# 30hours/blah2

Measured on AMD Instinct MI355X. Metric: CPIs/s, higher is better.
Workload: dtype f32; 1 GPU; BASELINE configs[1]: 2 MS/s, 1 s CPI, +-256 Hz -> 513 Doppler x 411 delay bins, synthetic c32 IQ resident in HBM; chain=amb, fmt=c32, n_samples=2000000, fs=2000000, n_doppler_bins=513, n_delay_bins=411, n_corr=3898, fft_len=1024, n_seg=7, seg_len=576, doppler_kernel=tile16, prewarm_steps=252, range_kernel=wave1k, ring_batches=2, streams_per_gpu=1

## Files before the change

blah2_amd/csrc/capi.hip:

```cpp
#include "kernels.hpp"
#include "cfar_kernels.hpp"
#include "timing.hpp"

#include <algorithm>
#include <cmath>
#include <complex>
#include <cstdio>
#include <cstdlib>
#include <cstring>
#include <deque>
#include <map>
#include <mutex>
#include <set>
#include <string>
#include <vector>

using namespace blah2;

namespace {

thread_local std::string g_err;

int fail(int code, const std::string &msg)
{
// ... 33 lines not shown
  int32_t delayMin = 0, delayMax = 0, dopplerMin = 0, dopplerMax = 0;
  uint32_t fs = 0;
  int r3 = 8;
  RangePlan plan{};
  struct LagChunk { int32_t lag0, count, col0; };
  std::vector<LagChunk> chunks;
  int32_t maxChunk = 0;
  std::vector<int32_t> delayAxis;
  std::vector<double> dopplerAxis;
  hipStream_t stream = nullptr;
  int numCU = 256;
  int rangeGridForce = 0;
  int rangeGridLast = 0;
  void *h_pin = nullptr;
  size_t h_pin_bytes = 0;

  cf *d_tw = nullptr;
  cf *d_dopW = nullptr;
  double2 *d_dopW64 = nullptr;
  uint32_t *d_hotCount = nullptr;
  cf *d_R = nullptr;
  cf *d_map = nullptr;
  double *d_partSum = nullptr;
  uint32_t *d_tickets = nullptr;
  float *d_partMax = nullptr;
  double *d_metrics = nullptr;
  double *d_doppler = nullptr;
  void *d_in = nullptr;
  size_t d_in_bytes = 0;
  cf *d_rot = nullptr;
  blah2hip_hit_t *d_hits = nullptr;
  uint32_t *d_count = nullptr;
  uint32_t hitCap = 0;
  int dopTilesX = 0, dopTilesY = 0;
  int dopR3 = 0;
  int dopGridX = 0;
  int nParts = 0;
  int nTiles = 0;
  int dopForce = BLAH2HIP_DOP_AUTO;
  int lastDoppler = 0;
  int lastRange = 0;
  int rangeKernel = 0;
  int fftLenForce = 0;
  int cfar2dForce = 0;
  int dopGridForce = 0;
  int dopGridLast = 0, dopTilesLast = 0;
// ... 303 lines not shown
  const bool out7 = a.plan.nDelay <= 7 * 64;
  auto kern = shortx ? (out7 ? rangeps_kernel<In, true, true> : rangeps_kernel<In, true, false>)
                     : (out7 ? rangeps_kernel<In, false, true> : rangeps_kernel<In, false, false>);
  LDSCFG(kern, lds);
  const int grid = std::min<int>(a.nPulses, range_grid_cap(h, lds, RANGEPS_WAVES, 12));
  hipLaunchKernelGGL(kern, dim3(grid), dim3(64 * RANGEPS_WAVES), lds, st, a, in);
  HIPCHK(hipGetLastError());
  h->lastRange = BLAH2HIP_RANGE_PS;
  return BLAH2HIP_OK;
}

template <class In> int launch_range(blah2hip_amb_s *h, const RangeArgs &a, In in, hipStream_t st)
{
  if (use_wave_range(h, a.nPulses)) return launch_rangew_t(h, a, in, st);
  if (use_wave1k_range(h, a.nPulses)) return launch_rangew1k_t(h, a, in, st);
  if (use_ps_range(h, a.nPulses)) return launch_rangeps_t(h, a, in, st);
  switch (h->r3) {
  case 4: return launch_range8_t<2>(h, a, in, st);
  case 8: return launch_range_t<8>(h, a, in, st);
  default: return launch_range_t<16>(h, a, in, st);
  }
}

int upload_range_table(blah2hip_amb_s *h)
{
  const int F = (int)h->dims.fft_len;
  std::vector<cf> tw(F);
  for (int k = 0; k < F; k++) tw[k] = root_of_unity(k, F);
  if (h->d_tw) HIPCHK(hipFree(h->d_tw));
  h->d_tw = nullptr;
  HIPCHK(hipMalloc(&h->d_tw, F * sizeof(cf)));
  HIPCHK(hipMemcpy(h->d_tw, tw.data(), F * sizeof(cf), hipMemcpyHostToDevice));
  return BLAH2HIP_OK;
}

int tic(blah2hip_amb_s *h, int k, hipStream_t st)
{
  HIPCHK(h->timer.tic(k, st));
  return BLAH2HIP_OK;
}

int toc(blah2hip_amb_s *h, int k, hipStream_t st)
{
  HIPCHK(h->timer.toc(k, st));
  return BLAH2HIP_OK;
}
// ... 604 lines not shown
    HIPCHK(hipMemcpy(h->d_chirp, chirp.data(), chirp.size() * sizeof(cf), hipMemcpyHostToDevice));
    HIPCHK(hipMemcpy(h->d_bf, bf.data(), bf.size() * sizeof(cf), hipMemcpyHostToDevice));
  }
  return BLAH2HIP_OK;
  };
  const int rc = build();
  if (rc != BLAH2HIP_OK) {
    blah2hip_amb_destroy(h);
    return rc;
  }
  *out = h;
  return BLAH2HIP_OK;
}

int blah2hip_amb_destroy(blah2hip_amb_t h)
{
  if (!h) return BLAH2HIP_OK;
  (void)hipSetDevice(h->device);
  if (h->stream) (void)hipStreamSynchronize(h->stream);
  for (void *p : {(void *)h->d_tw, (void *)h->d_dopW, (void *)h->d_R, (void *)h->d_map,
                  (void *)h->d_partSum, (void *)h->d_partMax, (void *)h->d_tickets, (void *)h->d_metrics,
                  (void *)h->d_doppler, h->d_in, (void *)h->d_rot,
                  (void *)h->d_hits, (void *)h->d_count, (void *)h->d_sat, (void *)h->d_dtw, (void *)h->d_chirp,
                  (void *)h->d_bf, (void *)h->d_bfn, (void *)h->d_H, (void *)h->d_dopW64, (void *)h->d_hotCount, (void *)h->d_firK0})
    if (p) (void)hipFree(p);
  for (auto &t : h->alphaTables)
    if (t.d) (void)hipFree(t.d);
  if (h->h_pin) (void)hipHostFree(h->h_pin);
  leak_clear(h);
  h->timer.destroy();
  if (h->stream) (void)hipStreamDestroy(h->stream);
  delete h;
  return BLAH2HIP_OK;
}

int blah2hip_amb_get_dims(blah2hip_amb_t h, blah2hip_amb_dims_t *dims)
{
  if (!h || !dims) return fail(BLAH2HIP_ERR_INVALID, "NULL argument");
  *dims = h->dims;
  return BLAH2HIP_OK;
}

int blah2hip_amb_get_axes(blah2hip_amb_t h, int32_t *delay, double *doppler)
{
  if (!h) return fail(BLAH2HIP_ERR_INVALID, "NULL handle");
  if (delay) std::memcpy(delay, h->delayAxis.data(), h->delayAxis.size() * sizeof(int32_t));
  if (doppler) std::memcpy(doppler, h->dopplerAxis.data(), h->dopplerAxis.size() * sizeof(double));
// ... 89 lines not shown
int blah2hip_amb_get_info(blah2hip_amb_t h, int key, int64_t *value)
{
  if (!h || !value) return fail(BLAH2HIP_ERR_INVALID, "NULL argument");
  switch (key) {
  case BLAH2HIP_INFO_LAST_DOPPLER_KERNEL: *value = h->lastDoppler; return BLAH2HIP_OK;
  case BLAH2HIP_INFO_LAST_RANGE_KERNEL: *value = h->lastRange; return BLAH2HIP_OK;
  case BLAH2HIP_INFO_DOPPLER_FFT_LEN: *value = 256 * h->dopR3; return BLAH2HIP_OK;
  case BLAH2HIP_INFO_RANGE_GRID: *value = h->rangeGridLast; return BLAH2HIP_OK;
  case BLAH2HIP_INFO_NUM_CU: *value = h->numCU; return BLAH2HIP_OK;
  case BLAH2HIP_INFO_DOPPLER_GRID: *value = h->dopGridLast; return BLAH2HIP_OK;
  case BLAH2HIP_INFO_DOPPLER_TILES: *value = h->dopTilesLast; return BLAH2HIP_OK;
  case BLAH2HIP_INFO_LEAK_LAGS: *value = h->lastLeakLags; return BLAH2HIP_OK;
  case BLAH2HIP_INFO_LEAK_MAX_E12: *value = (int64_t)std::llround(h->lastLeakMax * 1e12); return BLAH2HIP_OK;
  case BLAH2HIP_INFO_HOT_COLUMNS: {
    *value = 0;
    if (!h->lastHot) return BLAH2HIP_OK;
    uint32_t n = 0;
    HIPCHK(hipSetDevice(h->device));
    HIPCHK(hipMemcpyAsync(&n, h->d_hotCount, sizeof(n), hipMemcpyDeviceToHost, h->lastHotStream));
    HIPCHK(hipStreamSynchronize(h->lastHotStream));
    *value = n;
    return BLAH2HIP_OK;
  }
  case BLAH2HIP_INFO_HOT_COLUMNS_MISSED: {
    *value = 0;
    if (!h->lastHot) return BLAH2HIP_OK;
    std::vector<uint32_t> n(h->lastHotCpis);
    HIPCHK(hipSetDevice(h->device));
    HIPCHK(hipMemcpyAsync(n.data(), h->d_hotCount + h->dims.max_batch, n.size() * sizeof(uint32_t), hipMemcpyDeviceToHost,
                          h->lastHotStream));
    HIPCHK(hipStreamSynchronize(h->lastHotStream));
    for (uint32_t v : n) *value = std::max<int64_t>(*value, v);
    return BLAH2HIP_OK;
  }
  default: return fail(BLAH2HIP_ERR_INVALID, "unknown info key");
  }
}

int blah2hip_amb_process_dev(blah2hip_amb_t h, int fmt, const void *d_x, const void *d_y,
                             uint32_t n_cpi, uint64_t cpi_stride, void *d_map, double *d_metrics,
                             void *stream)
{
  if (!h) return fail(BLAH2HIP_ERR_INVALID, "NULL handle");
  if (n_cpi == 0 || n_cpi > h->dims.max_batch) return fail(BLAH2HIP_ERR_INVALID, "n_cpi outside [1, max_batch]");
  if (fmt != BLAH2HIP_FMT_C32 && fmt != BLAH2HIP_FMT_I16 && fmt != BLAH2HIP_FMT_F16 && fmt != BLAH2HIP_FMT_I16X_C32Y)
    return fail(BLAH2HIP_ERR_INVALID, "unknown sample format");
// ... 19 lines not shown
  if (h->leakMode != 0 && !h->inLeakCal && !fused) {
    const int rid = predict_range(h, (int)(n_cpi * nD)), did = pick_doppler(h, n_cpi);
    auto it = h->leak.find(rid * 64 + did);
    if (it == h->leak.end()) {
      blah2hip_amb_s::LeakCal cal;
      const int rcc = leak_calibrate(h, rid, did, st, &cal);
      if (rcc) return rcc;
      it = h->leak.emplace(rid * 64 + did, cal).first;
    }
    h->lastLeakMax = it->second.maxAbs;
    if (it->second.nLags > 0 && (it->second.active || h->leakMode == 2)) leak = &it->second;
  }
  if (!h->inLeakCal) h->lastLeakLags = leak ? leak->nLags : 0;

  RangeArgs ra;
  ra.plan = h->plan;
  ra.tw = h->d_tw;
  ra.out = h->d_R;
  ra.cpiStride = (int64_t)cpi_stride;
  ra.nPulses = (int32_t)(n_cpi * nD);

  const int32_t m2 = h->dopplerMin + h->dopplerMax;
  int rc;
  if (m2 != 0) {
    const size_t plane = (size_t)h->dims.n_samples;
    if (!h->d_rot) HIPCHK(hipMalloc(&h->d_rot, 2 * plane * h->dims.max_batch * sizeof(cf)));
    cf *xo = h->d_rot, *yo = h->d_rot + plane * h->dims.max_batch;
    const uint32_t nrot = h->dims.n_used;
    dim3 grid(std::min<uint32_t>((nrot + 255) / 256, 2048), n_cpi);
    if ((rc = tic(h, BLAH2HIP_K_ROTATE, st))) return rc;
    if (fmt == BLAH2HIP_FMT_C32) {
      InC32 in{(const cf *)d_x, (const cf *)d_y};
      hipLaunchKernelGGL(rotate_kernel<InC32>, grid, dim3(256), 0, st, in, xo, yo,
                         (int64_t)cpi_stride, (int64_t)plane, nrot, m2, h->fs);
    } else if (fmt == BLAH2HIP_FMT_F16) {
      InF16 in{(const _Float16 *)d_x, (const _Float16 *)d_y};
      hipLaunchKernelGGL(rotate_kernel<InF16>, grid, dim3(256), 0, st, in, xo, yo,
                         (int64_t)cpi_stride, (int64_t)plane, nrot, m2, h->fs);
    } else if (fmt == BLAH2HIP_FMT_I16X_C32Y) {
      InI16C32 in{(const int16_t *)d_x, (const cf *)d_y};
      hipLaunchKernelGGL(rotate_kernel<InI16C32>, grid, dim3(256), 0, st, in, xo, yo,
                         (int64_t)cpi_stride, (int64_t)plane, nrot, m2, h->fs);
    } else {
      InI16 in{(const int16_t *)d_x};
      hipLaunchKernelGGL(rotate_kernel<InI16>, grid, dim3(256), 0, st, in, xo, yo,
                         (int64_t)cpi_stride, (int64_t)plane, nrot, m2, h->fs);
// ... 13 lines not shown
    using W = WgFft<16>;
    const size_t lds = (size_t)(W::A_ELEMS + W::B_ELEMS) * sizeof(cf);
    LDSCFG(taps_spectrum_kernel, lds);
    hipLaunchKernelGGL(taps_spectrum_kernel, dim3(n_cpi), dim3(256), lds, st, h->firW, h->firBins, h->d_tw, h->d_H, h->d_firK0);
    RangeFirArgs fa;
    fa.plan = h->plan;
    fa.plan.delayMin = h->chunks[0].lag0; fa.plan.nDelay = h->chunks[0].count; fa.plan.colOff = h->chunks[0].col0;
    fa.tw = h->d_tw; fa.out = h->d_R; fa.cpiStride = (int64_t)cpi_stride; fa.nPulses = (int32_t)(n_cpi * nD);
    fa.H = h->d_H; fa.N = h->dims.n_samples; fa.w = h->firW; fa.nBins = h->firBins; fa.k0 = h->d_firK0;
    const size_t ldsf = lds + 240 * sizeof(cf);
    const int grid = std::min<int>(fa.nPulses, range_grid_cap(h, ldsf, 4, 8));
    if (fmt == BLAH2HIP_FMT_C32) {
      InC32 in{(const cf *)d_x, (const cf *)d_y};
      LDSCFG(range_fir_kernel<InC32>, ldsf);
      hipLaunchKernelGGL(range_fir_kernel<InC32>, dim3(grid), dim3(256), ldsf, st, fa, in);
    } else {
      InI16 in{(const int16_t *)d_x};
      LDSCFG(range_fir_kernel<InI16>, ldsf);
      hipLaunchKernelGGL(range_fir_kernel<InI16>, dim3(grid), dim3(256), ldsf, st, fa, in);
    }
    HIPCHK(hipGetLastError());
    h->lastRange = BLAH2HIP_RANGE_FIR;
    if ((rc = toc(h, BLAH2HIP_K_RANGE, st))) return rc;
  } else {
    if ((rc = tic(h, BLAH2HIP_K_RANGE, st))) return rc;
    for (const auto &ck : h->chunks) {
      ra.plan.delayMin = ck.lag0; ra.plan.nDelay = ck.count; ra.plan.colOff = ck.col0;
      if (fmt == BLAH2HIP_FMT_C32) {
        InC32 in{(const cf *)d_x, (const cf *)d_y};
        rc = launch_range(h, ra, in, st);
      } else if (fmt == BLAH2HIP_FMT_F16) {
        InF16 in{(const _Float16 *)d_x, (const _Float16 *)d_y};
        rc = launch_range(h, ra, in, st);
      } else if (fmt == BLAH2HIP_FMT_I16X_C32Y) {
        InI16C32 in{(const int16_t *)d_x, (const cf *)d_y};
        rc = launch_range(h, ra, in, st);
      } else {
        InI16 in{(const int16_t *)d_x};
        rc = launch_range(h, ra, in, st);
      }
      if (rc) return rc;
    }
    if ((rc = toc(h, BLAH2HIP_K_RANGE, st))) return rc;
  }

  DopplerArgs da;
  da.R = h->d_R;
  da.map = map;
  da.W = h->d_dopW;
  da.tw = h->d_dtw;
  da.chirp = h->d_chirp;
  da.bf = h->d_bf;
  da.bfn = h->d_bfn;
  da.partSum = h->d_partSum;
  da.partMax = h->d_partMax;
  da.nD = (int32_t)nD;
  da.nDelay = (int32_t)nDelay;
  da.nTiles = h->nTiles;
  int nPartsUsed = 0, dopGrid = 0, dopTiles = 0;
  if ((rc = tic(h, BLAH2HIP_K_DOPPLER, st))) return rc;
  const int which = pick_doppler(h, n_cpi);
  switch (which) {
  case BLAH2HIP_DOP_TILE8:
  case BLAH2HIP_DOP_TILE8K:
  case BLAH2HIP_DOP_TILE16WG:
  case BLAH2HIP_DOP_TILE16: {
    const int ncol = (which == BLAH2HIP_DOP_TILE8 || which == BLAH2HIP_DOP_TILE8K) ? 8 : 16;
    const int grid = (int)((nDelay + ncol - 1) / ncol);
    if (which == BLAH2HIP_DOP_TILE16) {
      const size_t lds = (size_t)DOPT1K_LDS_ELEMS * sizeof(cf);
      const int wgs = (int)std::min<int64_t>((int64_t)grid * n_cpi, h->dopGridForce ? h->dopGridForce : h->numCU);
      dopGrid = wgs; dopTiles = grid * (int)n_cpi;
      LDSCFG(doppler_tile1k_kernel<16>, lds);
      hipLaunchKernelGGL(doppler_tile1k_kernel<16>, dim3(wgs), dim3(1024), lds, st, da, (int)n_cpi);
    } else if (which == BLAH2HIP_DOP_TILE8K) {
      const size_t lds = (size_t)dopt1k_lds_elems<8>() * sizeof(cf);
      const int wgs = (int)std::min<int64_t>((int64_t)grid * n_cpi, h->dopGridForce ? h->dopGridForce : 2 * h->numCU);
      dopGrid = wgs; dopTiles = grid * (int)n_cpi;
      LDSCFG(doppler_tile1k_kernel<8>, lds);
      hipLaunchKernelGGL(doppler_tile1k_kernel<8>, dim3(wgs), dim3(512), lds, st, da, (int)n_cpi);
    } else if (ncol == 16) {
      const size_t lds = (size_t)dopt_lds_elems<16>() * sizeof(cf);
      const int wgs = (int)std::min<int64_t>((int64_t)grid * n_cpi, h->dopGridForce ? h->dopGridForce : h->numCU);
      dopGrid = wgs; dopTiles = grid * (int)n_cpi;
      LDSCFG(doppler_tile_kernel<16>, lds);
// ... 753 lines not shown
```

blah2_amd/csrc/kernels.hpp:

```cpp
#pragma once

#include <hip/hip_runtime.h>

#include "blah2hip.h"
#include "range_core.hpp"
#include "fft_wg8.hpp"
#include "fft_wave.hpp"
#include "fft_wave2.hpp"
#include "fft_wave1k.hpp"
#include "bufload.hpp"
#include "trace.hpp"

namespace blah2 {

#ifndef RANGE8_WAVES_PER_SIMD
#define RANGE8_WAVES_PER_SIMD 3
#endif
struct RangeArgs {
  RangePlan plan;
  const cf *tw;
  cf *out;
  int64_t cpiStride;
  int32_t nPulses;
};
// ... 410 lines not shown
  const int cnt = min(p.segLen, p.nCorr - s0);
  const b2_v4i xd = make_rsrc(B::xp(in, pulseBase + s0), cnt * CX::STRIDE);
  const b2_v4i yd = make_rsrc(B::yp(in, pulseBase), p.nCorr * CY::STRIDE);
  int vx[1] = {t * CX::STRIDE};
  int vy[NV];
#pragma unroll
  for (int j = 0; j < NV; j++) vy[j] = (s0 + p.delayMin + t) * CY::STRIDE + j * 4096;
  typename CX::raw xr[NX];
  typename CY::raw yr[NY];
  bufload_chan<CX, STEPX, NX, true>(xr, xd, vx);
  bufload_chan<CY, STEPY, NY, false>(yr, yd, vy);
  bufwait<NY + NX - 16, 16>(xr);
  if constexpr (NX == 32) bufwait<NY, 16>(xr + 16);
  else bufwait<NY, 8>(xr + 16);
#pragma unroll
  for (int k = 0; k < NX; k++) v[k] = CX::cvt(xr[k]);
  bufwait<NY - 16, 16>(yr);
  if constexpr (NY == 32) bufwait<0, 16>(yr + 16);
  else { bufwait<4, 8>(yr + 16); bufwait<0, 4>(yr + 24); }
#pragma unroll
  for (int k = 0; k < NY; k++) yv[k] = CY::cvt(yr[k]);
}

template <int NC>
__device__ __forceinline__ void store_lags_w(cf *out, const RangePlan &p, int cpi, int pulse, int t, const cf *v)
{
  const int jt = t + (p.colOff & 15);
  cf *o = out + (((int64_t)cpi * p.nTilesOut + (p.colOff >> 4) + (jt >> 4)) * p.nDoppler + pulse) * 16 + (jt & 15);
  const int64_t step = (int64_t)p.nDoppler * 64;
  int rem = p.nDelay - t;
  int nd = p.nDelay;
  asm volatile("" : "+v"(rem), "+s"(nd));
#pragma unroll
  for (int c = 0; c < NC; c++) {
    if (64 * c >= nd) break;
#if defined(RW_NO_STORE)
    if (64 * c < rem && p.scale == 12345.f) *o = cmake(v[c].x * p.scale, v[c].y * p.scale);
#else
    if (64 * c < rem) *o = cmake(v[c].x * p.scale, v[c].y * p.scale);
#endif
    o += step;
  }
}

#ifdef RANGEW_TRACE
#define RW_T(k) { const uint64_t now_ = __builtin_amdgcn_s_memtime(); tr[k] += now_ - t0_; t0_ = now_; }
#else
#define RW_T(k)
#endif

#ifndef RANGEW_WAVES
#define RANGEW_WAVES 8
#endif
template <class In, bool SHORTW, bool OUT7 = SHORTW>
__global__ __launch_bounds__(64 * RANGEW_WAVES, RANGEW_WAVES_PER_SIMD) void rangew_kernel(RangeArgs a, In in)
{
  using W = WaveFft;
  extern __shared__ __attribute__((aligned(16))) char smem[];
  cf *table = reinterpret_cast<cf *>(smem);
  const int t = threadIdx.x & 63;
  const int wave = __builtin_amdgcn_readfirstlane(threadIdx.x >> 6);
  cf *X = table + W::TW_ELEMS + wave * W::X_ELEMS;
// ... 71 lines not shown
  const int s0 = s * p.segLen;
  const int cnt = live ? min(p.segLen, p.nCorr - s0) : 0;
  const __amdgpu_buffer_rsrc_t d = make_rsrc_b(BufLoad<In>::xp(in, pulseBase + s0), cnt * CX::STRIDE);
#pragma unroll
  for (int k = 0; k < NX; k++) rx[k] = RawBuiltin<CX>::ld(d, t * CX::STRIDE, k * 64 * CX::STRIDE);
}
template <class In, int K0 = 0>
__device__ __forceinline__ void w1k_issue_y(const In &in, const RangePlan &p, int64_t pulseBase, int s, int t, bool live,
                                            typename RawBuiltin<typename BufLoad<In>::Y>::raw *ry)
{
  using CY = typename BufLoad<In>::Y;
  const __amdgpu_buffer_rsrc_t d = make_rsrc_b(BufLoad<In>::yp(in, pulseBase), live ? p.nCorr * CY::STRIDE : 0);
  constexpr int STEP = 64 * CY::STRIDE, NV = (15 * STEP >> 12) + 1;
  int vb[NV];
#pragma unroll
  for (int j = 0; j < NV; j++) {
    vb[j] = (s * p.segLen + p.delayMin + t) * CY::STRIDE + j * 4096;
    asm volatile("" : "+v"(vb[j]));
  }
#pragma unroll
  for (int k = K0; k < 16; k++) ry[k] = RawBuiltin<CY>::ld(d, vb[(k * STEP) >> 12] + ((k * STEP) & 4095), 0);
}

template <class In, bool SHORTX, bool OUT7, bool REUSE = false>
__global__ __launch_bounds__(64 * RANGEW1K_WAVES, RANGEW1K_WAVES_PER_SIMD) void rangew1k_kernel(RangeArgs a, In in)
{
  static_assert(!REUSE || SHORTX, "");
  using W = Wave1kFft;
  using RX = RawBuiltin<typename BufLoad<In>::X>;
  using RY = RawBuiltin<typename BufLoad<In>::Y>;
  constexpr int NX = SHORTX ? 9 : 16;
  extern __shared__ __attribute__((aligned(16))) char smem[];
  cf *table = reinterpret_cast<cf *>(smem);
  const int t = threadIdx.x & 63;
  const int wave = __builtin_amdgcn_readfirstlane(threadIdx.x >> 6);
  cf *X = table + W::TW_ELEMS + wave * W::X_ELEMS;
  W::fill_table(threadIdx.x, 64 * RANGEW1K_WAVES, a.tw, table);
  __syncthreads();
  W::Tw w;
  W::load_twiddles(t, a.tw, table, w);
  const RangePlan p = a.plan;
  const int stride = gridDim.x * RANGEW1K_WAVES;
  int pulse = blockIdx.x * RANGEW1K_WAVES + wave;
  if (pulse >= a.nPulses) return;
  int cpi = pulse / p.nDoppler;
  int i = pulse - cpi * p.nDoppler;
  int64_t base = (int64_t)cpi * a.cpiStride + (int64_t)i * p.nCorr;
  int s = 0;
  typename RX::raw rx[NX];
  typename RY::raw ry[16];
  cf acc[16];
#pragma unroll
  for (int e = 0; e < 16; e++) acc[e] = cmake(0.f, 0.f);
  w1k_issue_x<In, NX>(in, p, base, 0, t, true, rx);
  w1k_issue_y<In>(in, p, base, 0, t, true, ry);
#ifdef RANGEW_TRACE
  uint64_t tr[6] = {0, 0, 0, 0, 0, 0}, t0_ = __builtin_amdgcn_s_memtime();
#endif
  for (;;) {
    int ns = s + 1, npulse = pulse, ncpi = cpi, ni = i;
    int64_t nbase = base;
    if (ns == p.nSeg) {
      ns = 0;
      npulse = pulse + stride;
      ncpi = npulse / p.nDoppler;
      ni = npulse - ncpi * p.nDoppler;
      nbase = (int64_t)ncpi * a.cpiStride + (int64_t)ni * p.nCorr;
    }
    const bool more = npulse < a.nPulses;
    cf v[16];
    RW_T(0)
#pragma unroll
    for (int k = 0; k < NX; k++) v[k] = RX::cvt(rx[k]);
#ifdef RANGEW_TRACE
    asm volatile("" : "+v"(v[0].x), "+v"(v[NX - 1].y));
#endif
    RW_T(1)
    W::s1<-1, NX>(v, w);
    __builtin_amdgcn_sched_barrier(0);
    w1k_issue_x<In, NX>(in, p, nbase, ns, t, more, rx);
    __builtin_amdgcn_sched_barrier(0);
    W::finish<-1>(t, v, w, X);
#ifdef RANGEW_TRACE
    asm volatile("" : "+v"(v[0].x));
#endif
    RW_T(2)
    cf yin[16], yv[16];
#pragma unroll
    for (int k = 0; k < 16; k++) yin[k] = RY::cvt(ry[k]);
#ifdef RANGEW_TRACE
    asm volatile("" : "+v"(yin[0].x), "+v"(yin[15].y));
#endif
// ... 1 lines not shown
    W::s1_nd<-1>(yv, yin, w);
    W::finish<-1>(t, yv, w, X);
#pragma unroll
    for (int e = 0; e < 16; e++) acc[e] = cmacc(acc[e], yv[e], v[e]);
    __builtin_amdgcn_sched_barrier(0);
    if constexpr (REUSE) {
      if (ns != 0) {
#pragma unroll
        for (int k = 0; k < 7; k++) ry[k] = ry[9 + k];
        w1k_issue_y<In, 7>(in, p, nbase, ns, t, more, ry);
      } else {
        w1k_issue_y<In>(in, p, nbase, ns, t, more, ry);
      }
    } else {
      w1k_issue_y<In>(in, p, nbase, ns, t, more, ry);
    }
    __builtin_amdgcn_sched_barrier(0);
#ifdef RANGEW_TRACE
    asm volatile("" : "+v"(acc[0].x));
#endif
    RW_T(4)
    if (ns == 0) {
      W::template transform<+1, 16, OUT7>(t, acc, w, X);
      store_lags_w<OUT7 ? 7 : 16>(a.out, p, cpi, i, t, acc);
#ifdef RANGEW_TRACE
      RW_T(5)
      if (!more) {
        if (t == 0) trace_finish("rangew1k", tr, blockIdx.x == 0 && threadIdx.x == 0);
        break;
      }
#else
      if (!more) break;
#endif
#pragma unroll
      for (int e = 0; e < 16; e++) acc[e] = cmake(0.f, 0.f);
      pulse = npulse;
      cpi = ncpi;
      i = ni;
    }
    s = ns;
    base = nbase;
  }
}

#ifdef B2_RANGEW1K_GLDS
constexpr int RANGEG_WAVES = 16;
typedef __attribute__((address_space(3))) void b2_lds_void;
template <bool SHORTX, bool OUT7>
__global__ __launch_bounds__(64 * RANGEG_WAVES, 4) void rangew1k_glds_kernel(RangeArgs a, InC32 in)
{
  using W = Wave1kFft;
  constexpr int NX = SHORTX ? 9 : 16, PX = SHORTX ? 5 : 8;
  extern __shared__ __attribute__((aligned(16))) char smem[];
  cf *table = reinterpret_cast<cf *>(smem);
  const int t = threadIdx.x & 63;
  const int wave = __builtin_amdgcn_readfirstlane(threadIdx.x >> 6);
  cf *X = table + W::TW_ELEMS + wave * W::X_ELEMS;
  W::fill_table(threadIdx.x, 64 * RANGEG_WAVES, a.tw, table);
  __syncthreads();
  W::Tw w;
  W::load_twiddles(t, a.tw, table, w);
  const RangePlan p = a.plan;
  const int stride = gridDim.x * RANGEG_WAVES;
  int pulse = blockIdx.x * RANGEG_WAVES + wave;
  if (pulse >= a.nPulses) return;
// ... 757 lines not shown
    double sacc = 0.0;
    float m = 0.f;
    for (int i = 0; i < NCOL; i++) { sacc += ssum[i]; m = fmaxf(m, smax[i]); }
    const size_t part = (size_t)cpi * subsPerCpi + sub;
    __hip_atomic_store(a.partSum + part, sacc, __ATOMIC_RELAXED, __HIP_MEMORY_SCOPE_AGENT);
    __hip_atomic_store(a.partMax + part, m, __ATOMIC_RELAXED, __HIP_MEMORY_SCOPE_AGENT);
    int last = 0;
    if (a.tickets) {
      asm volatile("s_waitcnt vmcnt(0)" ::: "memory");
      const unsigned tk = __hip_atomic_fetch_add(a.tickets + cpi, 1u, __ATOMIC_RELAXED, __HIP_MEMORY_SCOPE_AGENT);
      last = tk == (unsigned)subsPerCpi - 1u;
      if (last) __hip_atomic_store(a.tickets + cpi, 0u, __ATOMIC_RELAXED, __HIP_MEMORY_SCOPE_AGENT);
    }
    lastWg = last;
  }
  __syncthreads();
  if (lastWg) metrics_finish_256(a.partSum, a.partMax, subsPerCpi, cpi, (double)nD * (double)a.nDelay, a.metrics, ssum, smax);
  DS_T(6)
#ifdef DOPW_TRACE
  if (t == 0) trace_finish("dops", tr, blockIdx.x == 0);
#endif
}
#undef DS_T

constexpr int DOPW_NCOL = 8;
constexpr int DOPW_MAX_ND = 1025;
constexpr int DOPW_RS = WaveFft::X_ELEMS + 2;
static_assert(DOPW_RS % 8 == 2, "");
constexpr int DOPW_CHIRP_ELEMS = 1088;
constexpr int DOPW_LDS_ELEMS = WaveFft::TW_ELEMS + DOPW_NCOL * DOPW_RS + DOPW_CHIRP_ELEMS;
__global__ __launch_bounds__(64 * DOPW_NCOL, 2) void doppler_tilew_kernel(DopplerArgs a, int nCpi)
{
#ifdef DOPW_TRACE
  uint64_t tr[8] = {0, 0, 0, 0, 0, 0, 0, 0}, t0_ = __builtin_amdgcn_s_memtime();
#define DW_T(k) { const uint64_t now_ = __builtin_amdgcn_s_memtime(); tr[k] += now_ - t0_; t0_ = now_; }
#else
#define DW_T(k)
#endif
  using W = WaveFft;
  constexpr int NCOL = DOPW_NCOL, NT = 64 * NCOL, SH = 3;
  constexpr int NR = 17;
  constexpr int NRP = 9;
  extern __shared__ __attribute__((aligned(16))) char smem[];
  __shared__ double wsum[NCOL];
  __shared__ float wmax[NCOL];
  cf *table = reinterpret_cast<cf *>(smem);
// ... 809 lines not shown
```

include/blah2hip.h:

```cpp
#ifndef BLAH2HIP_H
#define BLAH2HIP_H

#include <stddef.h>
#include <stdint.h>

#ifdef __cplusplus
extern "C" {
#endif

#define BLAH2HIP_OK 0
#define BLAH2HIP_ERR_INVALID (-1)
#define BLAH2HIP_ERR_HIP (-2)
#define BLAH2HIP_ERR_UNSUPPORTED (-3)
#define BLAH2HIP_ERR_UNDERFLOW (-4)
#define BLAH2HIP_ERR_NO_DEVICE (-5)
#define BLAH2HIP_ERR_CAPACITY (-6)

#define BLAH2HIP_FMT_C32 0
#define BLAH2HIP_FMT_I16 1
#define BLAH2HIP_FMT_F16 2
#define BLAH2HIP_FMT_I16X_C32Y 3

typedef struct blah2hip_amb_s *blah2hip_amb_t;
typedef struct blah2hip_clutter_s *blah2hip_clutter_t;
// ... 45 lines not shown
#define BLAH2HIP_OPT_HOT_COLUMNS 8
#define BLAH2HIP_CFAR2D_AUTO 0
#define BLAH2HIP_CFAR2D_TILE 1
#define BLAH2HIP_CFAR2D_SAT 2
#define BLAH2HIP_CFAR2D_STREAM 3
#define BLAH2HIP_DOP_AUTO 0
#define BLAH2HIP_DOP_TILE8 1
#define BLAH2HIP_DOP_TILE16 2
#define BLAH2HIP_DOP_TILEM 3
#define BLAH2HIP_DOP_COLUMN 4
#define BLAH2HIP_DOP_DIRECT 5
#define BLAH2HIP_DOP_TILEW 6
#define BLAH2HIP_DOP_TILEW2 7
#define BLAH2HIP_DOP_TILE16WG 8
#define BLAH2HIP_DOP_TILEW4 11
#define BLAH2HIP_DOP_TILE8K 10
#define BLAH2HIP_DOP_SUB4 9
#define BLAH2HIP_RANGE_E16 1
#define BLAH2HIP_RANGE_E8 2
#define BLAH2HIP_RANGE_WAVE 3
#define BLAH2HIP_RANGE_WAVE1K 5
#define BLAH2HIP_RANGE_FIR 7
#define BLAH2HIP_RANGE_PS 6
int blah2hip_amb_set_option(blah2hip_amb_t h, int option, int64_t value);
#define BLAH2HIP_INFO_LAST_DOPPLER_KERNEL 1
#define BLAH2HIP_INFO_LAST_RANGE_KERNEL 2
#define BLAH2HIP_INFO_DOPPLER_FFT_LEN 3
#define BLAH2HIP_INFO_RANGE_GRID 4
#define BLAH2HIP_INFO_NUM_CU 5
#define BLAH2HIP_INFO_DOPPLER_GRID 6
#define BLAH2HIP_INFO_LEAK_LAGS 8
#define BLAH2HIP_INFO_LEAK_MAX_E12 9
#define BLAH2HIP_INFO_HOT_COLUMNS 10
#define BLAH2HIP_INFO_HOT_COLUMNS_MISSED 11
#define BLAH2HIP_INFO_DOPPLER_TILES 7
int blah2hip_amb_get_info(blah2hip_amb_t h, int key, int64_t *value);

int blah2hip_amb_process_c64(blah2hip_amb_t h, const double *x, const double *y, uint32_t n,
                             float *map_out, double *metrics);
int blah2hip_amb_process_c32(blah2hip_amb_t h, const float *x, const float *y, uint32_t n,
                             float *map_out, double *metrics);
int blah2hip_amb_process_i16(blah2hip_amb_t h, const int16_t *iq, uint32_t n, float *map_out,
                             double *metrics);

int blah2hip_amb_process_dev(blah2hip_amb_t h, int fmt, const void *d_x, const void *d_y,
                             uint32_t n_cpi, uint64_t cpi_stride, void *d_map, double *d_metrics,
                             void *stream);
int blah2hip_amb_read_last(blah2hip_amb_t h, uint32_t cpi, float *map_out, double *metrics);
int blah2hip_amb_db_dev(blah2hip_amb_t h, const void *d_map, const double *d_metrics, uint32_t n_cpi,
                        float *d_db, void *stream);

int blah2hip_cfar1d_dev(blah2hip_amb_t h, const void *d_map, const double *d_metrics,
                        uint32_t n_cpi, double pfa, int32_t n_guard, int32_t n_train,
                        int32_t min_delay, double min_doppler, blah2hip_hit_t *d_hits,
                        uint32_t cap, uint32_t *d_count, void *stream);
int blah2hip_cfar1d_prepare(blah2hip_amb_t h, double pfa, int32_t n_train);
int blah2hip_cfar1d_process(blah2hip_amb_t h, uint32_t cpi, double pfa, int32_t n_guard,
// ... 118 lines not shown
```

Measured before the change: 112,700 CPIs/s.

## Fuse wave1k range FFT and tile16 Doppler into one persistent work-queue kernel

Adds a persistent kernel that takes range-compression and Doppler work items from an atomic counter. Doppler items for a CPI spin-wait on per-CPI pulse-completion counters, and range results are stored with agent-scope atomics so they become visible. The intent is to overlap the range and Doppler stages and drop the separate kernel launch and idle tail between them. A small fold kernel then reduces the per-column metric partials. The costs are spin-waiting with a timeout fallback, atomic-store overhead, LDS pressure, and a different metric reduction order.

```diff
diff --git a/blah2_amd/csrc/capi.hip b/blah2_amd/csrc/capi.hip
--- a/blah2_amd/csrc/capi.hip
+++ b/blah2_amd/csrc/capi.hip
@@ -79,6 +79,11 @@
   cf *d_R = nullptr;
   cf *d_map = nullptr;
   double *d_partSum = nullptr;
+  uint32_t *d_fusedCtl = nullptr;
+  double *d_s2Sum = nullptr;
+  float *d_s2Max = nullptr;
+  int fusedTables = -1;
+  bool lastFused = false;
   uint32_t *d_tickets = nullptr;
   float *d_partMax = nullptr;
   double *d_metrics = nullptr;
@@ -428,6 +433,51 @@
   }
 }
 
+int predict_range(const blah2hip_amb_s *h, int nPulses);
+int pick_doppler(const blah2hip_amb_s *h, uint32_t n_cpi);
+bool use_fused_range_doppler(blah2hip_amb_s *h, uint32_t n_cpi)
+{
+  if (h->rangeKernel != 0 || h->dopForce != BLAH2HIP_DOP_AUTO || h->inLeakCal || h->firW) return false;
+  if (h->chunks.size() != 1 || h->dopplerMin + h->dopplerMax != 0) return false;
+  const int nD = (int)h->dims.n_doppler_bins;
+  if (predict_range(h, (int)n_cpi * nD) != BLAH2HIP_RANGE_WAVE1K || pick_doppler(h, n_cpi) != BLAH2HIP_DOP_TILE16) return false;
+  if (h->fusedTables < 0) {
+    std::vector<cf> dtw, chirp, bf, bfn;
+    doppler_tables(nD, h->dopR3, dtw, chirp, bf, bfn);
+    bool same = (int)h->dims.fft_len == 1024 && dtw.size() == 1024;
+    for (int k = 0; same && k < 1024; k++) {
+      const cf r = root_of_unity(k, 1024);
+      same = std::memcmp(&r, &dtw[k], sizeof(cf)) == 0;
+    }
+    h->fusedTables = same ? 1 : 0;
+  }
+  return h->fusedTables == 1;
+}
+
+template <class In> int launch_fused_t(blah2hip_amb_s *h, FusedArgs &f, In in, hipStream_t st)
+{
+  const size_t lds = (size_t)FUSED_LDS_ELEMS * sizeof(cf);
+  const bool shortx = f.r.plan.segLen <= 9 * 64;
+  const bool out7 = f.r.plan.nDelay <= 7 * 64;
+  const bool reuse = f.r.plan.segLen == 9 * 64 && f.r.plan.nDelay <= 7 * 64 + 1;
+  auto kern = reuse ? (out7 ? range_doppler_fused_kernel<In, true, true, true> : range_doppler_fused_kernel<In, true, false, true>)
+              : shortx ? (out7 ? range_doppler_fused_kernel<In, true, true, false> : range_doppler_fused_kernel<In, true, false, false>)
+                       : (out7 ? range_doppler_fused_kernel<In, false, true, false> : range_doppler_fused_kernel<In, false, false, false>);
+  LDSCFG(kern, lds);
+  int perCU = 0;
+  HIPCHK(hipOccupancyMaxActiveBlocksPerMultiprocessor(&perCU, kern, 256, lds));
+  if (perCU < 1) return fail(BLAH2HIP_ERR_HIP, "range_doppler_fused_kernel: no resident workgroup");
+  perCU = std::min(perCU, 3);
+  const int grid = perCU * h->numCU;
+  f.lag = (grid * FUSED_PULSES + (int)f.d.nD - 1) / (int)f.d.nD + 2;
+  HIPCHK(hipMemsetAsync(f.ctl, 0, (2 + (size_t)f.nCpi) * sizeof(uint32_t), st));
+  hipLaunchKernelGGL(kern, dim3(grid), dim3(256), lds, st, f, in);
+  HIPCHK(hipGetLastError());
+  h->rangeGridLast = grid;
+  h->dopGridLast = grid;
+  return BLAH2HIP_OK;
+}
+
 int upload_range_table(blah2hip_amb_s *h)
 {
   const int F = (int)h->dims.fft_len;
@@ -1078,7 +1128,8 @@
                   (void *)h->d_partSum, (void *)h->d_partMax, (void *)h->d_tickets, (void *)h->d_metrics,
                   (void *)h->d_doppler, h->d_in, (void *)h->d_rot,
                   (void *)h->d_hits, (void *)h->d_count, (void *)h->d_sat, (void *)h->d_dtw, (void *)h->d_chirp,
-                  (void *)h->d_bf, (void *)h->d_bfn, (void *)h->d_H, (void *)h->d_dopW64, (void *)h->d_hotCount, (void *)h->d_firK0})
+                  (void *)h->d_bf, (void *)h->d_bfn, (void *)h->d_H, (void *)h->d_dopW64, (void *)h->d_hotCount, (void *)h->d_firK0,
+                  (void *)h->d_fusedCtl, (void *)h->d_s2Sum, (void *)h->d_s2Max})
     if (p) (void)hipFree(p);
   for (auto &t : h->alphaTables)
     if (t.d) (void)hipFree(t.d);
@@ -1214,6 +1265,16 @@
     *value = n;
     return BLAH2HIP_OK;
   }
+  case BLAH2HIP_INFO_FUSED_TIMEOUTS: {
+    *value = 0;
+    if (!h->lastFused) return BLAH2HIP_OK;
+    uint32_t n = 0;
+    HIPCHK(hipSetDevice(h->device));
+    HIPCHK(hipDeviceSynchronize());
+    HIPCHK(hipMemcpy(&n, h->d_fusedCtl + 1, sizeof(uint32_t), hipMemcpyDeviceToHost));
+    *value = n;
+    return BLAH2HIP_OK;
+  }
   case BLAH2HIP_INFO_HOT_COLUMNS_MISSED: {
     *value = 0;
     if (!h->lastHot) return BLAH2HIP_OK;
@@ -1279,6 +1340,8 @@
 
   const int32_t m2 = h->dopplerMin + h->dopplerMax;
   int rc;
+  const bool fusedRD = !fused && use_fused_range_doppler(h, n_cpi);
+  h->lastFused = fusedRD;
   if (m2 != 0) {
     const size_t plane = (size_t)h->dims.n_samples;
     if (!h->d_rot) HIPCHK(hipMalloc(&h->d_rot, 2 * plane * h->dims.max_batch * sizeof(cf)));
@@ -1338,6 +1401,32 @@
     HIPCHK(hipGetLastError());
     h->lastRange = BLAH2HIP_RANGE_FIR;
     if ((rc = toc(h, BLAH2HIP_K_RANGE, st))) return rc;
+  } else if (fusedRD) {
+    if ((rc = tic(h, BLAH2HIP_K_RANGE, st))) return rc;
+    const size_t tiles = (nDelay + 15) / 16, s2 = (size_t)h->dims.max_batch * tiles * 256;
+    if (!h->d_fusedCtl) HIPCHK(hipMalloc(&h->d_fusedCtl, (2 + (size_t)h->dims.max_batch) * sizeof(uint32_t)));
+    if (!h->d_s2Sum) HIPCHK(hipMalloc(&h->d_s2Sum, s2 * sizeof(double)));
+    if (!h->d_s2Max) HIPCHK(hipMalloc(&h->d_s2Max, s2 * sizeof(float)));
+    FusedArgs f;
+    f.r = ra;
+    f.r.plan.delayMin = h->chunks[0].lag0; f.r.plan.nDelay = h->chunks[0].count; f.r.plan.colOff = h->chunks[0].col0;
+    f.d.R = h->d_R; f.d.map = map; f.d.W = h->d_dopW; f.d.tw = h->d_dtw; f.d.chirp = h->d_chirp; f.d.bf = h->d_bf; f.d.bfn = h->d_bfn;
+    f.d.partSum = h->d_partSum; f.d.partMax = h->d_partMax;
+    f.d.nD = (int32_t)nD; f.d.nDelay = (int32_t)nDelay; f.d.nTiles = h->nTiles;
+    f.ctl = h->d_fusedCtl; f.s2Sum = h->d_s2Sum; f.s2Max = h->d_s2Max;
+    f.nCpi = (int32_t)n_cpi; f.lag = 0;
+    if (fmt == BLAH2HIP_FMT_C32) {
+      rc = launch_fused_t(h, f, InC32{(const cf *)d_x, (const cf *)d_y}, st);
+    } else if (fmt == BLAH2HIP_FMT_F16) {
+      rc = launch_fused_t(h, f, InF16{(const _Float16 *)d_x, (const _Float16 *)d_y}, st);
+    } else if (fmt == BLAH2HIP_FMT_I16X_C32Y) {
+      rc = launch_fused_t(h, f, InI16C32{(const int16_t *)d_x, (const cf *)d_y}, st);
+    } else {
+      rc = launch_fused_t(h, f, InI16{(const int16_t *)d_x}, st);
+    }
+    if (rc) return rc;
+    h->lastRange = BLAH2HIP_RANGE_FUSED;
+    if ((rc = toc(h, BLAH2HIP_K_RANGE, st))) return rc;
   } else {
     if ((rc = tic(h, BLAH2HIP_K_RANGE, st))) return rc;
     for (const auto &ck : h->chunks) {
@@ -1376,7 +1465,16 @@
   int nPartsUsed = 0, dopGrid = 0, dopTiles = 0;
   if ((rc = tic(h, BLAH2HIP_K_DOPPLER, st))) return rc;
   const int which = pick_doppler(h, n_cpi);
-  switch (which) {
+  switch (fusedRD ? -1 : which) {
+  case -1: {
+    const int tiles = (int)((nDelay + 15) / 16);
+    hipLaunchKernelGGL(fused_metrics_fold_kernel, dim3(tiles, n_cpi), dim3(64), 0, st, h->d_s2Sum, h->d_s2Max, (int)nDelay,
+                       h->d_partSum, h->d_partMax);
+    dopTiles = (int)((nDelay + 3) / 4) * (int)n_cpi;
+    dopGrid = h->dopGridLast;
+    nPartsUsed = tiles;
+    break;
+  }
   case BLAH2HIP_DOP_TILE8:
   case BLAH2HIP_DOP_TILE8K:
   case BLAH2HIP_DOP_TILE16WG:
diff --git a/blah2_amd/csrc/kernels.hpp b/blah2_amd/csrc/kernels.hpp
--- a/blah2_amd/csrc/kernels.hpp
+++ b/blah2_amd/csrc/kernels.hpp
@@ -456,7 +456,7 @@
   for (int k = 0; k < NY; k++) yv[k] = CY::cvt(yr[k]);
 }
 
-template <int NC>
+template <int NC, bool SC1 = false>
 __device__ __forceinline__ void store_lags_w(cf *out, const RangePlan &p, int cpi, int pulse, int t, const cf *v)
 {
   const int jt = t + (p.colOff & 15);
@@ -471,7 +471,11 @@
 #if defined(RW_NO_STORE)
     if (64 * c < rem && p.scale == 12345.f) *o = cmake(v[c].x * p.scale, v[c].y * p.scale);
 #else
-    if (64 * c < rem) *o = cmake(v[c].x * p.scale, v[c].y * p.scale);
+    if (64 * c < rem) {
+      const cf d = cmake(v[c].x * p.scale, v[c].y * p.scale);
+      if constexpr (SC1) __hip_atomic_store(reinterpret_cast<uint64_t *>(o), __builtin_bit_cast(uint64_t, d), __ATOMIC_RELAXED, __HIP_MEMORY_SCOPE_AGENT);
+      else *o = d;
+    }
 #endif
     o += step;
   }
@@ -589,27 +593,16 @@
   for (int k = K0; k < 16; k++) ry[k] = RawBuiltin<CY>::ld(d, vb[(k * STEP) >> 12] + ((k * STEP) & 4095), 0);
 }
 
-template <class In, bool SHORTX, bool OUT7, bool REUSE = false>
-__global__ __launch_bounds__(64 * RANGEW1K_WAVES, RANGEW1K_WAVES_PER_SIMD) void rangew1k_kernel(RangeArgs a, In in)
+template <class In, bool SHORTX, bool OUT7, bool REUSE, bool SC1>
+__device__ __forceinline__ void w1k_walk(const RangeArgs &a, const In &in, const Wave1kFft::Tw &w, cf *X, int t, int pulse,
+                                         int stride, int end)
 {
   static_assert(!REUSE || SHORTX, "");
   using W = Wave1kFft;
   using RX = RawBuiltin<typename BufLoad<In>::X>;
   using RY = RawBuiltin<typename BufLoad<In>::Y>;
   constexpr int NX = SHORTX ? 9 : 16;
-  extern __shared__ __attribute__((aligned(16))) char smem[];
-  cf *table = reinterpret_cast<cf *>(smem);
-  const int t = threadIdx.x & 63;
-  const int wave = __builtin_amdgcn_readfirstlane(threadIdx.x >> 6);
-  cf *X = table + W::TW_ELEMS + wave * W::X_ELEMS;
-  W::fill_table(threadIdx.x, 64 * RANGEW1K_WAVES, a.tw, table);
-  __syncthreads();
-  W::Tw w;
-  W::load_twiddles(t, a.tw, table, w);
   const RangePlan p = a.plan;
-  const int stride = gridDim.x * RANGEW1K_WAVES;
-  int pulse = blockIdx.x * RANGEW1K_WAVES + wave;
-  if (pulse >= a.nPulses) return;
   int cpi = pulse / p.nDoppler;
   int i = pulse - cpi * p.nDoppler;
   int64_t base = (int64_t)cpi * a.cpiStride + (int64_t)i * p.nCorr;
@@ -634,7 +627,7 @@
       ni = npulse - ncpi * p.nDoppler;
       nbase = (int64_t)ncpi * a.cpiStride + (int64_t)ni * p.nCorr;
     }
-    const bool more = npulse < a.nPulses;
+    const bool more = npulse < end;
     cf v[16];
     RW_T(0)
 #pragma unroll
@@ -682,7 +675,7 @@
     RW_T(4)
     if (ns == 0) {
       W::template transform<+1, 16, OUT7>(t, acc, w, X);
-      store_lags_w<OUT7 ? 7 : 16>(a.out, p, cpi, i, t, acc);
+      store_lags_w<OUT7 ? 7 : 16, SC1>(a.out, p, cpi, i, t, acc);
 #ifdef RANGEW_TRACE
       RW_T(5)
       if (!more) {
@@ -701,6 +694,26 @@
     s = ns;
     base = nbase;
   }
+}
+
+template <class In, bool SHORTX, bool OUT7, bool REUSE = false>
+__global__ __launch_bounds__(64 * RANGEW1K_WAVES, RANGEW1K_WAVES_PER_SIMD) void rangew1k_kernel(RangeArgs a, In in)
+{
+  static_assert(!REUSE || SHORTX, "");
+  using W = Wave1kFft;
+  extern __shared__ __attribute__((aligned(16))) char smem[];
+  cf *table = reinterpret_cast<cf *>(smem);
+  const int t = threadIdx.x & 63;
+  const int wave = __builtin_amdgcn_readfirstlane(threadIdx.x >> 6);
+  cf *X = table + W::TW_ELEMS + wave * W::X_ELEMS;
+  W::fill_table(threadIdx.x, 64 * RANGEW1K_WAVES, a.tw, table);
+  __syncthreads();
+  W::Tw w;
+  W::load_twiddles(t, a.tw, table, w);
+  const int stride = gridDim.x * RANGEW1K_WAVES;
+  int pulse = blockIdx.x * RANGEW1K_WAVES + wave;
+  if (pulse >= a.nPulses) return;
+  w1k_walk<In, SHORTX, OUT7, REUSE, false>(a, in, w, X, t, pulse, stride, a.nPulses);
 }
 
 #ifdef B2_RANGEW1K_GLDS
@@ -1504,6 +1517,206 @@
 #endif
 }
 #undef DS_T
+
+constexpr int FUSED_PULSES = 16;
+constexpr int FUSED_LDS_ELEMS = Wave1kFft::TW_ELEMS + 1024 + 4 * DOPT_PITCH;
+static_assert(Wave1kFft::X_ELEMS <= DOPT_PITCH, "");
+struct FusedArgs {
+  RangeArgs r;
+  DopplerArgs d;
+  uint32_t *ctl;
+  double *s2Sum;
+  float *s2Max;
+  int32_t nCpi, lag;
+};
+
+template <class In, bool SHORTX, bool OUT7, bool REUSE>
+__global__ __launch_bounds__(256, 3) void range_doppler_fused_kernel(FusedArgs f, In in)
+{
+  using K = Wave1kFft;
+  constexpr int NCOL = 4, T = 64, NR = 9, NT = 256, SH = 2, S = FUSED_PULSES;
+  extern __shared__ __attribute__((aligned(16))) char smem[];
+  __shared__ int item;
+  cf *table = reinterpret_cast<cf *>(smem);
+  cf *bfL = table + K::TW_ELEMS;
+  cf *lds = bfL + 1024;
+  const int tid = threadIdx.x;
+  const int wave = __builtin_amdgcn_readfirstlane(tid >> 6), t = tid & 63;
+  const int nD = f.d.nD;
+  const int nPulses = f.r.nPulses;
+  const int RI = (nPulses + S - 1) / S;
+  const int D = (f.d.nDelay + NCOL - 1) / NCOL;
+  const int tilesPerCpi = (f.d.nDelay + 15) / 16;
+  const int total = RI + f.nCpi * D;
+  K::fill_table(tid, NT, f.r.tw, table);
+#pragma unroll
+  for (int j = 0; j < 1024 / NT; j++) bfL[tid + NT * j] = f.d.bfn[tid + NT * j];
+  K::Tw tw;
+  K::load_twiddles(t, f.r.tw, table, tw);
+  auto first_dop = [&](int d) { return min(((d + f.lag + 1) * nD + S - 1) / S, RI) + d * D; };
+  for (;;) {
+    __syncthreads();
+    if (tid == 0) item = (int)__hip_atomic_fetch_add(f.ctl, 1u, __ATOMIC_RELAXED, __HIP_MEMORY_SCOPE_AGENT);
+    __syncthreads();
+    const int tk = __builtin_amdgcn_readfirstlane(item);
+    if (tk >= total) break;
+    int lo = -1, hi = f.nCpi - 1;
+    while (lo < hi) {
+      const int mid = (lo + hi + 1) >> 1;
+      if (first_dop(mid) <= tk) lo = mid; else hi = mid - 1;
+    }
+    const int fd = lo < 0 ? 0 : first_dop(lo);
+    if (lo < 0 || tk >= fd + D) {
+      const int r = lo < 0 ? tk : tk - (lo + 1) * D;
+      const int p0 = r * S + wave, end = min(r * S + S, nPulses);
+      if (p0 < end) {
+        w1k_walk<In, SHORTX, OUT7, REUSE, true>(f.r, in, tw, lds + wave * K::X_ELEMS, t, p0, NCOL, end);
+        asm volatile("s_waitcnt vmcnt(0)" ::: "memory");
+        if (t == 0) {
+          const int n = (end - 1 - p0) / NCOL + 1, c0 = p0 / nD, cl = (p0 + NCOL * (n - 1)) / nD;
+          const int n0 = c0 == cl ? n : ((c0 + 1) * nD - 1 - p0) / NCOL + 1;
+          __hip_atomic_fetch_add(f.ctl + 2 + c0, (uint32_t)n0, __ATOMIC_RELAXED, __HIP_MEMORY_SCOPE_AGENT);
+          if (n0 < n) __hip_atomic_fetch_add(f.ctl + 2 + cl, (uint32_t)(n - n0), __ATOMIC_RELAXED, __HIP_MEMORY_SCOPE_AGENT);
+        }
+      }
+      continue;
+    }
+    const int cpi = lo, sub = tk - fd;
+    const int col0 = sub * NCOL;
+    if (tid == 0) {
+      bool ok = false;
+      for (int n = 0; n < (1 << 22); n++) {
+        if (__hip_atomic_load(f.ctl + 2 + cpi, __ATOMIC_RELAXED, __HIP_MEMORY_SCOPE_AGENT) >= (uint32_t)nD) { ok = true; break; }
+        __builtin_amdgcn_s_sleep(2);
+      }
+      if (!ok) {
+        __hip_atomic_fetch_add(f.ctl + 1, 1u, __ATOMIC_RELAXED, __HIP_MEMORY_SCOPE_AGENT);
+        __builtin_amdgcn_fence(__ATOMIC_ACQUIRE, "agent");
+        asm volatile("s_waitcnt vmcnt(0)" ::: "memory");
+      }
+    }
+    __syncthreads();
+    __builtin_amdgcn_fence(__ATOMIC_ACQUIRE, "wavefront");
+    const int cells = nD * NCOL;
+    cf nt[NR];
+    {
+      const uint64_t *Rt = reinterpret_cast<const uint64_t *>(f.d.R + rmap_index(nD, f.d.nTiles, cpi, 0, col0));
+#pragma unroll
+      for (int j = 0; j < NR; j++) {
+        const int idx = tid + NT * j;
+        const int c = idx & (NCOL - 1), row = idx >> SH;
+        nt[j] = __builtin_bit_cast(cf, __hip_atomic_load(Rt + (idx < cells ? row * 16 + c : 0), __ATOMIC_RELAXED, __HIP_MEMORY_SCOPE_AGENT));
+      }
+    }
+    int tq = t;
+    asm volatile("" : "+v"(tq));
+    cf ch[NR];
+    int oidx[NR], ridx[NR];
+#pragma unroll
+    for (int k = 0; k < NR; k++) {
+      const int i = tq + T * k;
+      ridx[k] = min(i, nD - 1);
+      const cf c = f.d.chirp[min(i, nD - 1)];
+      ch[k] = cmake(i < nD ? c.x : 0.f, i < nD ? c.y : 0.f);
+      int o = i - (nD / 2 + 1);
+      if (o < 0) o += nD;
+      oidx[k] = i < nD ? o : DOPT_PITCH - 1;
+    }
+    cf *region = lds + wave * DOPT_PITCH;
+    {
+      cf *dst = lds + (tid & (NCOL - 1)) * DOPT_PITCH + (tid >> SH);
+#pragma unroll
+      for (int j = 0; j < NR; j++)
+        if (tid + NT * j < cells) dst[T * j] = nt[j];
+    }
+    __syncthreads();
+    cf v[16];
+    const cf r0 = region[0];
+#pragma unroll
+    for (int k = 0; k < NR; k++) v[k] = cmul(csub(region[ridx[k]], r0), ch[k]);
+    __builtin_amdgcn_wave_barrier();
+    K::transform<-1, 9>(t, v, tw, region);
+#pragma unroll
+    for (int e = 0; e < 16; e++) v[e] = cmul(v[e], bfL[e * T + t]);
+    __builtin_amdgcn_wave_barrier();
+    K::transform<+1>(t, v, tw, region);
+    __builtin_amdgcn_wave_barrier();
+#pragma unroll
+    for (int c = 0; c < NR; c++) {
+      cf d = cmul(v[c], ch[c]);
+      if (c == 0 && t == 0) d = cmake(d.x + (float)nD * r0.x, d.y + (float)nD * r0.y);
+      region[oidx[c]] = d;
+    }
+    __syncthreads();
+    double lsum = 0.0;
+    float lmax = 0.f;
+    cf *mapb = f.d.map + (size_t)cpi * nD * f.d.nDelay + col0;
+    const int ncol = min(NCOL, f.d.nDelay - col0);
+    {
+      const int c = tid & (NCOL - 1), o0 = tid >> SH;
+      const cf *src = lds + c * DOPT_PITCH + o0;
+      cf *dstg = mapb + (size_t)o0 * f.d.nDelay + c;
+      const size_t gstep = (size_t)T * f.d.nDelay;
+#pragma unroll
+      for (int j = 0; j < NR; j++) {
+        const bool ok = tid + NT * j < cells && c < ncol;
+        const cf d = src[min(T * j, nD - 1 - o0)];
+        if (ok) dstg[gstep * j] = d;
+        const float db = db_of(d);
+        lsum += ok ? (double)db : 0.0;
+        lmax = ok ? fmaxf(lmax, db) : lmax;
+      }
+    }
+    lsum += __shfl_xor(lsum, 8);
+    lmax = fmaxf(lmax, __shfl_xor(lmax, 8));
+    lsum += __shfl_xor(lsum, 4);
+    lmax = fmaxf(lmax, __shfl_xor(lmax, 4));
+    if ((t & 12) == 0) {
+      const size_t e = (((size_t)cpi * tilesPerCpi + (sub >> 2)) * 16 + 4 * wave + (t >> 4)) * 16 + 4 * (sub & 3) + (t & 3);
+      f.s2Sum[e] = lsum;
+      f.s2Max[e] = lmax;
+    }
+  }
+}
+
+__global__ __launch_bounds__(64) void fused_metrics_fold_kernel(const double *s2Sum, const float *s2Max, int nDelay,
+                                                                double *partSum, float *partMax)
+{
+  __shared__ double wsum[16];
+  __shared__ float wmax[16];
+  const int tile = blockIdx.x, cpi = blockIdx.y, tilesPerCpi = gridDim.x, w = threadIdx.x;
+  if (w < 16) {
+    const size_t base = (((size_t)cpi * tilesPerCpi + tile) * 16 + w) * 16;
+    double s[16];
+    float m[16];
+#pragma unroll
+    for (int c = 0; c < 16; c++) {
+      const bool live = tile * 16 + (c & ~3) < nDelay;
+      s[c] = live ? s2Sum[base + c] : 0.0;
+      m[c] = live ? s2Max[base + c] : 0.f;
+    }
+#pragma unroll
+    for (int off = 8; off > 0; off >>= 1) {
+      double n[16];
+      float nm[16];
+#pragma unroll
+      for (int c = 0; c < 16; c++) { n[c] = s[c] + s[c ^ off]; nm[c] = fmaxf(m[c], m[c ^ off]); }
+#pragma unroll
+      for (int c = 0; c < 16; c++) { s[c] = n[c]; m[c] = nm[c]; }
+    }
+    wsum[w] = s[0];
+    wmax[w] = m[0];
+  }
+  __syncthreads();
+  if (threadIdx.x == 0) {
+    double sacc = 0.0;
+    float mm = 0.f;
+    for (int i = 0; i < 16; i++) { sacc += wsum[i]; mm = fmaxf(mm, wmax[i]); }
+    const size_t part = (size_t)cpi * tilesPerCpi + tile;
+    partSum[part] = sacc;
+    partMax[part] = mm;
+  }
+}
 
 constexpr int DOPW_NCOL = 8;
 constexpr int DOPW_MAX_ND = 1025;
diff --git a/include/blah2hip.h b/include/blah2hip.h
--- a/include/blah2hip.h
+++ b/include/blah2hip.h
@@ -91,6 +91,7 @@
 #define BLAH2HIP_RANGE_WAVE1K 5
 #define BLAH2HIP_RANGE_FIR 7
 #define BLAH2HIP_RANGE_PS 6
+#define BLAH2HIP_RANGE_FUSED 8
 int blah2hip_amb_set_option(blah2hip_amb_t h, int option, int64_t value);
 #define BLAH2HIP_INFO_LAST_DOPPLER_KERNEL 1
 #define BLAH2HIP_INFO_LAST_RANGE_KERNEL 2
@@ -102,6 +103,7 @@
 #define BLAH2HIP_INFO_LEAK_MAX_E12 9
 #define BLAH2HIP_INFO_HOT_COLUMNS 10
 #define BLAH2HIP_INFO_HOT_COLUMNS_MISSED 11
+#define BLAH2HIP_INFO_FUSED_TIMEOUTS 12
 #define BLAH2HIP_INFO_DOPPLER_TILES 7
 int blah2hip_amb_get_info(blah2hip_amb_t h, int key, int64_t *value);
 
```

Result: slower. 97580 CPIs/s, median of 2 (-13.4%).
